# revdotcom/reverb

Measured on NVIDIA H100. Metric: rtfx_attention_rescoring_30s_chunks, higher is better.
Workload: dtype bf16

## Files before the change

reverb_b200/csrc/common.cuh:

```cuda
#pragma once
#include <cuda.h>
#include <cuda_bf16.h>
#include <cuda_runtime.h>
#include <stdint.h>
#include <stdio.h>
#include <string.h>

#include <atomic>

namespace rvb {

void set_error(const char* fmt, ...);
const char* last_error();

#define RVB_CHECK_CUDA(expr)                                                              \
  do {                                                                                    \
    cudaError_t _e = (expr);                                                              \
    if (_e != cudaSuccess) {                                                              \
      rvb::set_error("%s:%d CUDA error %d (%s) in %s", __FILE__, __LINE__, (int)_e,       \
                     cudaGetErrorString(_e), #expr);                                      \
      return -1;                                                                          \
    }                                                                                     \
  } while (0)

#define RVB_REQUIRE(cond, ...)                                                            \
  do {                                                                                    \
    if (!(cond)) {                                                                        \
      rvb::set_error(__VA_ARGS__);                                                        \
      return -2;                                                                          \
    }                                                                                     \
  } while (0)

#define RVB_CHECK_LAUNCH() RVB_CHECK_CUDA(cudaGetLastError())

extern std::atomic<unsigned long long> g_launch_count;
#define RVB_COUNT_LAUNCH() (rvb::g_launch_count.fetch_add(1, std::memory_order_relaxed))

typedef __nv_bfloat16 bf16;

struct DynSmemOptIn {
  static constexpr int kMaxDev = 64;
  std::atomic<size_t> cfg[kMaxDev];
  DynSmemOptIn() {
    for (auto& c : cfg) c.store(0);
  }
  template <typename K>
  int ensure(K kernel, size_t bytes) {
    if (bytes <= 48 * 1024) return 0;
    int dev = 0;
    RVB_CHECK_CUDA(cudaGetDevice(&dev));
    if (dev >= 0 && dev < kMaxDev && cfg[dev].load(std::memory_order_relaxed) >= bytes) return 0;
    RVB_CHECK_CUDA(cudaFuncSetAttribute(kernel, cudaFuncAttributeMaxDynamicSharedMemorySize, (int)bytes));
    if (dev >= 0 && dev < kMaxDev) cfg[dev].store(bytes, std::memory_order_relaxed);
    return 0;
  }
};

__device__ __forceinline__ float2 ffma2(float2 a, float2 b, float2 c) {
  return make_float2(fmaf(a.x, b.x, c.x), fmaf(a.y, b.y, c.y));
}

__device__ __forceinline__ float warp_sum(float v) {
#pragma unroll
  for (int o = 16; o > 0; o >>= 1) v += __shfl_xor_sync(0xffffffffu, v, o);
  return v;
}
__device__ __forceinline__ float warp_max(float v) {
#pragma unroll
  for (int o = 16; o > 0; o >>= 1) v = fmaxf(v, __shfl_xor_sync(0xffffffffu, v, o));
  return v;
}
__device__ __forceinline__ float silu_f(float x) { return x / (1.0f + __expf(-x)); }
__device__ __forceinline__ float sigmoid_f(float x) { return 1.0f / (1.0f + __expf(-x)); }
__device__ __forceinline__ float gelu_erf(float x) { return 0.5f * x * (1.0f + erff(x * 0.70710678118654752f)); }

static inline uint16_t f2bf(float f) {
  uint32_t u;
  memcpy(&u, &f, 4);
  if ((u & 0x7fffffffu) > 0x7f800000u) return (uint16_t)((u >> 16) | 0x40);
  u += 0x7fffu + ((u >> 16) & 1u);
  return (uint16_t)(u >> 16);
}

static inline float bf2f(uint16_t h) {
  uint32_t u = (uint32_t)h << 16;
  float f;
  memcpy(&f, &u, 4);
  return f;
}

__device__ __forceinline__ uint32_t pack_bf16x2(float lo, float hi) {
  __nv_bfloat162 t = __floats2bfloat162_rn(lo, hi);
  return *reinterpret_cast<uint32_t*>(&t);
}
__device__ __forceinline__ float2 unpack_bf16x2(uint32_t u) {
  __nv_bfloat162 t = *reinterpret_cast<__nv_bfloat162*>(&u);
  return __bfloat1622float2(t);
}

__device__ __forceinline__ uint32_t smem_u32(const void* p) {
  return static_cast<uint32_t>(__cvta_generic_to_shared(p));
}

__device__ __forceinline__ void mbar_init(uint64_t* bar, uint32_t count) {
  asm volatile("mbarrier.init.shared::cta.b64 [%0], %1;" ::"r"(smem_u32(bar)), "r"(count));
}
__device__ __forceinline__ void fence_barrier_init() {
  asm volatile("fence.mbarrier_init.release.cluster;" ::: "memory");
}
__device__ __forceinline__ void fence_proxy_async() {
  asm volatile("fence.proxy.async.shared::cta;" ::: "memory");
}
__device__ __forceinline__ void mbar_expect_tx(uint64_t* bar, uint32_t bytes) {
  asm volatile("mbarrier.arrive.expect_tx.shared::cta.b64 _, [%0], %1;" ::"r"(smem_u32(bar)), "r"(bytes)
               : "memory");
}
__device__ __forceinline__ void mbar_arrive(uint64_t* bar) {
  asm volatile("mbarrier.arrive.shared::cta.b64 _, [%0];" ::"r"(smem_u32(bar)) : "memory");
}
__device__ __forceinline__ uint32_t mbar_try_wait(uint64_t* bar, uint32_t parity) {
  uint32_t ok;
  asm volatile(
      "{\n"
      ".reg .pred p;\n"
      "mbarrier.try_wait.parity.shared::cta.b64 p, [%1], %2;\n"
      "selp.u32 %0, 1, 0, p;\n"
      "}\n"
      : "=r"(ok)
      : "r"(smem_u32(bar)), "r"(parity)
      : "memory");
  return ok;
}
__device__ __forceinline__ void mbar_wait(uint64_t* bar, uint32_t parity) {
  while (!mbar_try_wait(bar, parity)) {
  }
}

template <uint32_t N>
__device__ __forceinline__ void setmaxnreg_dec() {
  asm volatile("setmaxnreg.dec.sync.aligned.u32 %0;" ::"n"(N));
}
template <uint32_t N>
__device__ __forceinline__ void setmaxnreg_inc() {
  asm volatile("setmaxnreg.inc.sync.aligned.u32 %0;" ::"n"(N));
}

__device__ __forceinline__ void tma_prefetch_desc(const CUtensorMap* m) {
  asm volatile("prefetch.tensormap [%0];" ::"l"(reinterpret_cast<uint64_t>(m)) : "memory");
}
__device__ __forceinline__ void tma_load_4d(void* smem_dst, const CUtensorMap* m, uint64_t* bar, int c0, int c1,
                                            int c2, int c3) {
  asm volatile(
      "cp.async.bulk.tensor.4d.shared::cluster.global.mbarrier::complete_tx::bytes [%0], [%1, {%3, %4, %5, %6}], [%2];"
      ::"r"(smem_u32(smem_dst)),
      "l"(reinterpret_cast<uint64_t>(m)), "r"(smem_u32(bar)), "r"(c0), "r"(c1), "r"(c2), "r"(c3)
      : "memory");
}
__device__ __forceinline__ void tma_load_2d(void* smem_dst, const CUtensorMap* m, uint64_t* bar, int c0, int c1) {
  asm volatile(
      "cp.async.bulk.tensor.2d.shared::cluster.global.mbarrier::complete_tx::bytes [%0], [%1, {%3, %4}], [%2];"
      ::"r"(smem_u32(smem_dst)),
      "l"(reinterpret_cast<uint64_t>(m)), "r"(smem_u32(bar)), "r"(c0), "r"(c1)
      : "memory");
}

__device__ __forceinline__ void wgmma_fence() { asm volatile("wgmma.fence.sync.aligned;" ::: "memory"); }
__device__ __forceinline__ void wgmma_commit() { asm volatile("wgmma.commit_group.sync.aligned;" ::: "memory"); }
template <int N>
__device__ __forceinline__ void wgmma_wait() {
  asm volatile("wgmma.wait_group.sync.aligned %0;" ::"n"(N) : "memory");
}
template <int R>
__device__ __forceinline__ void wgmma_fence_regs(float* d) {
#pragma unroll
  for (int i = 0; i < R; ++i) asm volatile("" : "+f"(d[i])::"memory");
}
__device__ __forceinline__ void wgmma_m64n128k16_ss(float* d, uint64_t adesc, uint64_t bdesc, uint32_t accumulate) {
  asm volatile(
      "{\n"
      ".reg .pred p;\n"
      "setp.ne.b32 p, %66, 0;\n"
      "wgmma.mma_async.sync.aligned.m64n128k16.f32.bf16.bf16 "
      "{%0, %1, %2, %3, %4, %5, %6, %7, %8, %9, %10, %11, %12, %13, %14, %15, %16, %17, %18, %19, %20, %21, %22, %23, %24, %25, %26, %27, %28, %29, %30, %31, %32, %33, %34, %35, %36, %37, %38, %39, %40, %41, %42, %43, %44, %45, %46, %47, %48, %49, %50, %51, %52, %53, %54, %55, %56, %57, %58, %59, %60, %61, %62, %63}, %64, %65, p, 1, 1, 0, 0;\n"
      "}\n"
      : "+f"(d[0]), "+f"(d[1]), "+f"(d[2]), "+f"(d[3]), "+f"(d[4]), "+f"(d[5]), "+f"(d[6]), "+f"(d[7]), "+f"(d[8]), "+f"(d[9]), "+f"(d[10]), "+f"(d[11]), "+f"(d[12]), "+f"(d[13]), "+f"(d[14]), "+f"(d[15]), "+f"(d[16]), "+f"(d[17]), "+f"(d[18]), "+f"(d[19]), "+f"(d[20]), "+f"(d[21]), "+f"(d[22]), "+f"(d[23]), "+f"(d[24]), "+f"(d[25]), "+f"(d[26]), "+f"(d[27]), "+f"(d[28]), "+f"(d[29]), "+f"(d[30]), "+f"(d[31]), "+f"(d[32]), "+f"(d[33]), "+f"(d[34]), "+f"(d[35]), "+f"(d[36]), "+f"(d[37]), "+f"(d[38]), "+f"(d[39]), "+f"(d[40]), "+f"(d[41]), "+f"(d[42]), "+f"(d[43]), "+f"(d[44]), "+f"(d[45]), "+f"(d[46]), "+f"(d[47]), "+f"(d[48]), "+f"(d[49]), "+f"(d[50]), "+f"(d[51]), "+f"(d[52]), "+f"(d[53]), "+f"(d[54]), "+f"(d[55]), "+f"(d[56]), "+f"(d[57]), "+f"(d[58]), "+f"(d[59]), "+f"(d[60]), "+f"(d[61]), "+f"(d[62]), "+f"(d[63])
      : "l"(adesc), "l"(bdesc), "r"(accumulate)
      : "memory");
}
__device__ __forceinline__ void wgmma_m64n64k16_ss(float* d, uint64_t adesc, uint64_t bdesc, uint32_t accumulate) {
  asm volatile(
      "{\n"
      ".reg .pred p;\n"
      "setp.ne.b32 p, %34, 0;\n"
      "wgmma.mma_async.sync.aligned.m64n64k16.f32.bf16.bf16 "
      "{%0, %1, %2, %3, %4, %5, %6, %7, %8, %9, %10, %11, %12, %13, %14, %15, %16, %17, %18, %19, %20, %21, %22, %23, %24, %25, %26, %27, %28, %29, %30, %31}, %32, %33, p, 1, 1, 0, 0;\n"
      "}\n"
      : "+f"(d[0]), "+f"(d[1]), "+f"(d[2]), "+f"(d[3]), "+f"(d[4]), "+f"(d[5]), "+f"(d[6]), "+f"(d[7]), "+f"(d[8]), "+f"(d[9]), "+f"(d[10]), "+f"(d[11]), "+f"(d[12]), "+f"(d[13]), "+f"(d[14]), "+f"(d[15]), "+f"(d[16]), "+f"(d[17]), "+f"(d[18]), "+f"(d[19]), "+f"(d[20]), "+f"(d[21]), "+f"(d[22]), "+f"(d[23]), "+f"(d[24]), "+f"(d[25]), "+f"(d[26]), "+f"(d[27]), "+f"(d[28]), "+f"(d[29]), "+f"(d[30]), "+f"(d[31])
      : "l"(adesc), "l"(bdesc), "r"(accumulate)
      : "memory");
}
__device__ __forceinline__ void wgmma_m64n64k16_rs_tb(float* d, const uint32_t* a, uint64_t bdesc) {
  asm volatile(
      "wgmma.mma_async.sync.aligned.m64n64k16.f32.bf16.bf16 "
      "{%0, %1, %2, %3, %4, %5, %6, %7, %8, %9, %10, %11, %12, %13, %14, %15, %16, %17, %18, %19, %20, %21, %22, %23, %24, %25, %26, %27, %28, %29, %30, %31}, {%32, %33, %34, %35}, %36, 1, 1, 1, 1;\n"
      : "+f"(d[0]), "+f"(d[1]), "+f"(d[2]), "+f"(d[3]), "+f"(d[4]), "+f"(d[5]), "+f"(d[6]), "+f"(d[7]), "+f"(d[8]), "+f"(d[9]), "+f"(d[10]), "+f"(d[11]), "+f"(d[12]), "+f"(d[13]), "+f"(d[14]), "+f"(d[15]), "+f"(d[16]), "+f"(d[17]), "+f"(d[18]), "+f"(d[19]), "+f"(d[20]), "+f"(d[21]), "+f"(d[22]), "+f"(d[23]), "+f"(d[24]), "+f"(d[25]), "+f"(d[26]), "+f"(d[27]), "+f"(d[28]), "+f"(d[29]), "+f"(d[30]), "+f"(d[31])
      : "r"(a[0]), "r"(a[1]), "r"(a[2]), "r"(a[3]), "l"(bdesc)
      : "memory");
}

__device__ __forceinline__ uint64_t make_sw128_desc(uint32_t smem_addr) {
  uint64_t d = 0;
  d |= (uint64_t)((smem_addr >> 4) & 0x3FFF);
  d |= (uint64_t)(1024 >> 4) << 16;
  d |= (uint64_t)(1024 >> 4) << 32;
  d |= (uint64_t)1 << 62;
  return d;
}

__device__ __forceinline__ uint32_t cluster_ctarank() {
  uint32_t r;
  asm volatile("mov.u32 %0, %%cluster_ctarank;" : "=r"(r));
  return r;
}
__device__ __forceinline__ void cluster_sync_all() {
  asm volatile("barrier.cluster.arrive.release.aligned;\n\tbarrier.cluster.wait.acquire.aligned;" ::: "memory");
}

}
```

reverb_b200/csrc/gemm.cu:

```cuda
#include <cuda.h>
#include <stdlib.h>
#include <string.h>

#include <algorithm>
#include <mutex>
#include <vector>

#include "kernels.h"

namespace rvb {

static int g_gemm_impl = -1;
void set_gemm_impl(int impl) { g_gemm_impl = impl; }
int get_gemm_impl() {
  if (g_gemm_impl < 0) {
    const char* e = getenv("RVB_GEMM");
    g_gemm_impl = (e && strcmp(e, "simt") == 0) ? 1 : (e && strcmp(e, "narrow") == 0) ? 2 : 0;
  }
  return g_gemm_impl;
}

struct GemmKParams {
  int M, N, K, num_k_blocks;
  int tiles_n, num_tiles;
// ... 480 lines not shown
          }
          if (EPI == EPI_BF16_RELU) {
#pragma unroll
            for (int e = 0; e < 8; ++e) v[e] = fmaxf(v[e], 0.f);
          }
          if (EPI == EPI_BF16_GELU) {
#pragma unroll
            for (int e = 0; e < 8; ++e) v[e] = gelu_erf(v[e]);
          }
          if constexpr (EPI == EPI_BF16_RELPOS) {
            if (kcols) {
              const uint4 pv = *reinterpret_cast<const uint4*>(p.rp_pos + (long long)rp_t * p.rp_ldp + rp_hc + 8 * j);
              const float4 u0 = __ldg(reinterpret_cast<const float4*>(p.rp_u + rp_hc + 8 * j));
              const float4 u1 = __ldg(reinterpret_cast<const float4*>(p.rp_u + rp_hc + 8 * j) + 1);
              const float uu[8] = {u0.x, u0.y, u0.z, u0.w, u1.x, u1.y, u1.z, u1.w};
              const float4 v0 = __ldg(reinterpret_cast<const float4*>(p.rp_v + rp_hc + 8 * j));
              const float4 v1 = __ldg(reinterpret_cast<const float4*>(p.rp_v + rp_hc + 8 * j) + 1);
              const float2 p0 = unpack_bf16x2(pv.x), p1 = unpack_bf16x2(pv.y), p2 = unpack_bf16x2(pv.z), p3 = unpack_bf16x2(pv.w);
              const float pp[8] = {p0.x, p0.y, p1.x, p1.y, p2.x, p2.y, p3.x, p3.y};
              float kq[8];
#pragma unroll
              for (int e = 0; e < 8; ++e) {
                kq[e] = __bfloat162float(__float2bfloat16(v[e]));
                v[e] = kq[e] + pp[e];
              }
              rp_part[j] = uu[0] * kq[0] + uu[1] * kq[1] + uu[2] * kq[2] + uu[3] * kq[3] + uu[4] * kq[4] + uu[5] * kq[5] +
                           uu[6] * kq[6] + uu[7] * kq[7] + v0.x * pp[0] + v0.y * pp[1] + v0.z * pp[2] + v0.w * pp[3] +
                           v1.x * pp[4] + v1.y * pp[5] + v1.z * pp[6] + v1.w * pp[7];
            }
          }
          if (PAIR && part == 1) {
#pragma unroll
            for (int e = 0; e < 8; ++e) v[e] -= __bfloat162float(__float2bfloat16(v[e]));
          }
          if (p.debug_skip_epi == 3 && v[0] != 123.456f) continue;
          *reinterpret_cast<uint4*>(stage_u + lane * 32 + ((j ^ (lane & 7)) << 2)) =
              make_uint4(pack_bf16x2(v[0], v[1]), pack_bf16x2(v[2], v[3]), pack_bf16x2(v[4], v[5]),
                         pack_bf16x2(v[6], v[7]));
        }
        if (p.debug_skip_epi == 3) continue;
        __syncwarp();
#pragma unroll
        for (int it = 0; it < 8; ++it) {
          const int row = it * 4 + rsub;
          const uint4 u = *reinterpret_cast<const uint4*>(stage_u + row * 32 + ((slot ^ (row & 7)) << 2));
          if (ro[it] >= 0 && p.debug_skip_epi != 2)
            *reinterpret_cast<uint4*>(out + ro[it] + c + (PAIR ? part * p.out_split : 0)) = u;
        }
        __syncwarp();
        }
        if constexpr (EPI == EPI_BF16_RELPOS) {
          if (kcols && orow >= 0) {
            const int hh = rp_hc >> 6;
            p.rp_cb[((orow / p.rp_T) * p.rp_H + hh) * (long long)p.rp_T + rp_t] =
                ((rp_part[0] + rp_part[4]) + (rp_part[2] + rp_part[6])) + ((rp_part[1] + rp_part[5]) + (rp_part[3] + rp_part[7]));
          }
        }
      } else {
        for (int cc = c; cc < c + 64 && cc < c1; cc += 32) {
          if (n0_tile + cc >= p.N) break;
          uint32_t acc[32];
          acc_ld32<BN>(accs, arow, cc, acc);
          if (orow >= 0) store_chunk<EPI>(p, orow, n0_tile + cc, oshift, acc);
        }
      }
    }
  } else if ((EPI == EPI_RESID || EPI == EPI_F32) && p.f32_coalesced) {
    const int slot = lane & 7, rsub = lane >> 3;
    long long ro[8];
#pragma unroll
    for (int it = 0; it < 8; ++it) {
      const long long o = __shfl_sync(0xffffffffu, orow, it * 4 + rsub);
      ro[it] = (o >= 0) ? o * p.ldo + n0_tile - oshift + slot * 4 : -1;
    }
    float* out = reinterpret_cast<float*>(p.out);
    float4 r[8];
    if (EPI == EPI_RESID && n0_tile + c0 + slot * 4 + 4 <= p.N) {
#pragma unroll
      for (int it = 0; it < 8; ++it)
        if (ro[it] >= 0) r[it] = *reinterpret_cast<const float4*>(out + ro[it] + c0);
    }
#pragma unroll 1
    for (int c = c0; c < c1; c += 32) {
      if (n0_tile + c >= p.N) break;
      uint32_t acc[32];
      acc_ld32<BN>(accs, arow, c, acc);
      const int n = n0_tile + c + slot * 4;
      const bool vec = (n + 4 <= p.N);
      float4 rn[8];
      const bool pre_next = EPI == EPI_RESID && (c + 32 < c1) && (n + 32 + 4 <= p.N);
      if (pre_next) {
#pragma unroll
        for (int it = 0; it < 8; ++it)
          if (ro[it] >= 0) rn[it] = *reinterpret_cast<const float4*>(out + ro[it] + c + 32);
      }
      float4 b4 = make_float4(0.f, 0.f, 0.f, 0.f);
      if (p.bias != nullptr) {
        if (vec) {
          b4 = __ldg(reinterpret_cast<const float4*>(p.bias + n));
        } else {
          if (n + 0 < p.N) b4.x = __ldg(p.bias + n + 0);
          if (n + 1 < p.N) b4.y = __ldg(p.bias + n + 1);
          if (n + 2 < p.N) b4.z = __ldg(p.bias + n + 2);
        }
      }
#pragma unroll
      for (int j = 0; j < 8; ++j)
        *reinterpret_cast<uint4*>(stage + lane * 32 + ((j ^ (lane & 7)) << 2)) =
            make_uint4(acc[4 * j], acc[4 * j + 1], acc[4 * j + 2], acc[4 * j + 3]);
      __syncwarp();
#pragma unroll
      for (int it = 0; it < 8; ++it) {
        const int row = it * 4 + rsub;
        float4 v = *reinterpret_cast<const float4*>(stage + row * 32 + ((slot ^ (row & 7)) << 2));
        v.x += b4.x; v.y += b4.y; v.z += b4.z; v.w += b4.w;
        if (ro[it] < 0) continue;
        float* o = out + ro[it] + c;
        if (vec) {
          if (EPI == EPI_RESID) {
            r[it].x += p.alpha * v.x; r[it].y += p.alpha * v.y; r[it].z += p.alpha * v.z; r[it].w += p.alpha * v.w;
            *reinterpret_cast<float4*>(o) = r[it];
          } else {
            *reinterpret_cast<float4*>(o) = v;
          }
        } else {
          const float vv[4] = {v.x, v.y, v.z, v.w};
#pragma unroll
          for (int k = 0; k < 3; ++k)
            if (n + k < p.N) o[k] = (EPI == EPI_RESID) ? o[k] + p.alpha * vv[k] : vv[k];
        }
      }
      __syncwarp();
      if (pre_next) {
#pragma unroll
        for (int it = 0; it < 8; ++it) r[it] = rn[it];
      }
    }
  } else {
#pragma unroll 1
    for (int c = c0; c < c1; c += 32) {
      if (n0_tile + c >= p.N) break;
      uint32_t acc[32];
      acc_ld32<BN>(accs, arow, c, acc);
      if (orow >= 0) store_chunk<EPI>(p, orow, n0_tile + c, oshift, acc);
    }
  }
}

constexpr int kConsumerWGs = 2;
constexpr int kGemmThreads = 128 * (1 + kConsumerWGs);
constexpr int kProducerRegs = 40;
constexpr int kConsumerRegs = 232;

template <int BN>
struct GemmCfg {
  static constexpr int BM = 128;
  static constexpr int BK = 64;
  static constexpr int STAGES = 4;
  static constexpr uint32_t A_BYTES = BM * BK * 2;
  static constexpr uint32_t B_BYTES = BN * BK * 2;
  static constexpr uint32_t STAGE_BYTES = A_BYTES + B_BYTES;
  static constexpr uint32_t ACC_BYTES = BM * BN * 4;
  static constexpr uint32_t SMEM_BYTES = STAGES * STAGE_BYTES + ACC_BYTES + 4 * 4096  +
                                         256  + 1024 ;
};

template <int BN, int EPI, bool PAIR>
__global__ void __launch_bounds__(kGemmThreads, 1)
gemm_wg_kernel(const __grid_constant__ CUtensorMap tmA, const __grid_constant__ CUtensorMap tmB, const GemmKParams p) {
  using Cfg = GemmCfg<BN>;
  constexpr int STAGES = Cfg::STAGES;
  extern __shared__ uint8_t smem_raw[];
  uint8_t* smem = reinterpret_cast<uint8_t*>((reinterpret_cast<uintptr_t>(smem_raw) + 1023) & ~uintptr_t(1023));
  uint8_t* sA = smem;
  uint8_t* sB = smem + STAGES * Cfg::A_BYTES;
  float* accs = reinterpret_cast<float*>(smem + STAGES * Cfg::STAGE_BYTES);
  float* stage_epi = accs + Cfg::BM * BN;
  uint64_t* bars = reinterpret_cast<uint64_t*>(stage_epi + 4 * 1024);
  uint64_t* full = bars;
  uint64_t* empty = bars + STAGES;
  uint64_t* turn = bars + 2 * STAGES;
  uint64_t* accfree = turn + 2;

  const int warp = threadIdx.x >> 5;
  const int lane = threadIdx.x & 31;

  if (threadIdx.x == 0) {
    for (int i = 0; i < STAGES; ++i) {
      mbar_init(&full[i], 1);
      mbar_init(&empty[i], 4);
    }
    for (int w = 0; w < kConsumerWGs; ++w) {
      mbar_init(&turn[w], 128);
      mbar_init(&accfree[w], 128);
    }
    fence_barrier_init();
    tma_prefetch_desc(&tmA);
    tma_prefetch_desc(&tmB);
  }
  __syncthreads();
  const int nkb = p.num_k_blocks;

  if (warp < 4) {
    setmaxnreg_dec<kProducerRegs>();
    if (warp == 0 && lane == 0) {
      uint32_t stage = 0, phase = 0;
      for (int tile = blockIdx.x; tile < p.num_tiles; tile += gridDim.x) {
        if (!tile_active(p, tile, BN)) continue;
        TileCoord t = decode_tile(p, tile, BN);
        for (int kbx = 0; kbx < nkb; ++kbx) {
          const int seg = p.x3 ? kbx / p.kb_seg : 0;
          const int kb = kbx - seg * p.kb_seg;
          const int a_ofs = (seg == 1) ? p.a_lo_ofs : 0, w_ofs = (seg == 2) ? p.w_lo_ofs : 0;
          mbar_wait(&empty[stage], phase ^ 1);
          mbar_expect_tx(&full[stage], Cfg::STAGE_BYTES);
          if (p.conv_mode) {
            int tap = kb / p.conv_cblocks;
            int cb = kb - tap * p.conv_cblocks;
            int kh = tap / 3, kw = tap - kh * 3;
            tma_load_4d(sA + stage * Cfg::A_BYTES, &tmA, &full[stage], cb * 64 + a_ofs, 2 * t.f + kw, t.row0 + (kh >> 1),
                        t.b * 2 + (kh & 1));
          } else {
            tma_load_4d(sA + stage * Cfg::A_BYTES, &tmA, &full[stage], kb * 64 + a_ofs, t.row0, 0, 0);
          }
          tma_load_2d(sB + stage * Cfg::B_BYTES, &tmB, &full[stage], kb * 64 + w_ofs, t.n0);
          if (++stage == STAGES) {
            stage = 0;
            phase ^= 1;
          }
        }
      }
    }
  } else {
    setmaxnreg_inc<kConsumerRegs>();
    const int wg = (warp >> 2) - 1, wl = warp & 3;
    float* stage_w = stage_epi + wl * 1024;
    float acc[BN];
    int active = 0;
    for (int tile = blockIdx.x; tile < p.num_tiles; tile += gridDim.x) {
      if (!tile_active(p, tile, BN)) continue;
      const int i = active++;
      if (i % kConsumerWGs != wg) continue;
      TileCoord t = decode_tile(p, tile, BN);
      const uint32_t u0 = (uint32_t)i * (uint32_t)nkb;
      uint32_t stage = u0 % STAGES, phase = (u0 / STAGES) & 1;
      const uint32_t hand_parity = ((i - 1) >> 1) & 1;
#pragma unroll
      for (int e = 0; e < BN; ++e) acc[e] = 0.f;
      if (i > 0) mbar_wait(&turn[wg], hand_parity);
      int prev = -1;
      for (int kb = 0; kb < nkb; ++kb) {
        mbar_wait(&full[stage], phase);
        const uint64_t adesc = make_sw128_desc(smem_u32(sA + stage * Cfg::A_BYTES));
        const uint64_t bdesc = make_sw128_desc(smem_u32(sB + stage * Cfg::B_BYTES));
        constexpr uint64_t kHalfA = (Cfg::A_BYTES / 2) >> 4;
        wgmma_fence_regs<BN>(acc);
        wgmma_fence();
#pragma unroll
        for (int k = 0; k < 4; ++k) {
          if constexpr (BN == 128) {
            wgmma_m64n128k16_ss(acc, adesc + 2 * k, bdesc + 2 * k, 1u);
            wgmma_m64n128k16_ss(acc + BN / 2, adesc + kHalfA + 2 * k, bdesc + 2 * k, 1u);
          } else {
            wgmma_m64n64k16_ss(acc, adesc + 2 * k, bdesc + 2 * k, 1u);
            wgmma_m64n64k16_ss(acc + BN / 2, adesc + kHalfA + 2 * k, bdesc + 2 * k, 1u);
          }
        }
        wgmma_commit();
        wgmma_wait<1>();
        wgmma_fence_regs<BN>(acc);
        if (prev >= 0 && lane == 0) mbar_arrive(&empty[prev]);
        prev = (int)stage;
        if (++stage == STAGES) {
          stage = 0;
          phase ^= 1;
        }
      }
      mbar_arrive(&turn[wg ^ 1]);
      wgmma_wait<0>();
      wgmma_fence_regs<BN>(acc);
      if (prev >= 0 && lane == 0) mbar_arrive(&empty[prev]);
      if (i > 0) mbar_wait(&accfree[wg], hand_parity);
#pragma unroll
      for (int h = 0; h < 2; ++h) {
        const int r0 = h * 64 + wl * 16 + (lane >> 2);
#pragma unroll
        for (int j = 0; j < BN / 8; ++j) {
          const int c = 8 * j + 2 * (lane & 3);
#pragma unroll
          for (int e = 0; e < 2; ++e) {
            const int r = r0 + 8 * e;
            *reinterpret_cast<float2*>(accs + r * BN + ((((c >> 2)) ^ (r & 7)) << 2) + (c & 3)) =
                make_float2(acc[h * (BN / 2) + 4 * j + 2 * e], acc[h * (BN / 2) + 4 * j + 2 * e + 1]);
          }
        }
      }
      asm volatile("bar.sync %0, 128;" ::"r"(1 + wg) : "memory");
      drain_tile<BN, EPI, PAIR>(p, t, wl, lane, accs, 0, BN, stage_w);
      mbar_arrive(&accfree[wg ^ 1]);
    }
  }
}

__device__ __forceinline__ float load_a_elem(const GemmKParams& p, const TileCoord& t, int r, int k) {
  if (k >= p.K) return 0.0f;
  if (p.conv_mode) {
    int tp = t.row0 + r;
    if (tp >= p.conv_T2) return 0.0f;
    int tap = k / p.conv_C;
    int c = k - tap * p.conv_C;
    int kh = tap / 3, kw = tap - kh * 3;
    long long idx = (((long long)(t.b * 2 + (kh & 1)) * p.conv_T1h + (tp + (kh >> 1))) * p.conv_F1 + (2 * t.f + kw)) *
                        p.conv_C + c;
    return __bfloat162float(p.A[idx]);
  }
  int m = t.row0 + r;
  if (m >= p.M) return 0.0f;
  return __bfloat162float(p.A[(long long)m * p.lda + k]);
}

__global__ void __launch_bounds__(256) gemm_simt_kernel(const GemmKParams p) {
  __shared__ float sA[128][17];
  __shared__ float sW[32][17];
  __shared__ float sG[32][17];
  const bool glu = (p.act == ACT_GLU);
  for (int tile = blockIdx.x; tile < p.num_tiles; tile += gridDim.x) {
    TileCoord t = decode_tile(p, tile, 32);
    const int tx = threadIdx.x & 7, ty = threadIdx.x >> 3;
    const int wrow0 = glu ? 2 * t.n0 : t.n0;
    float acc[4][4], accg[4][4];
#pragma unroll
    for (int i = 0; i < 4; ++i)
#pragma unroll
      for (int j = 0; j < 4; ++j) acc[i][j] = accg[i][j] = 0.f;
    for (int k0 = 0; k0 < p.K; k0 += 16) {
      for (int e = threadIdx.x; e < 128 * 16; e += 256) {
        int r = e >> 4, kk = e & 15;
        sA[r][kk] = load_a_elem(p, t, r, k0 + kk);
      }
      for (int e = threadIdx.x; e < 32 * 16; e += 256) {
        int n = e >> 4, kk = e & 15;
        int gn = wrow0 + n, gk = k0 + kk;
        sW[n][kk] = (gn < p.N && gk < p.K) ? __bfloat162float(p.W[(long long)gn * p.ldw + gk]) : 0.f;
        sG[n][kk] = (glu && gn + 32 < p.N && gk < p.K) ? __bfloat162float(p.W[(long long)(gn + 32) * p.ldw + gk]) : 0.f;
      }
      __syncthreads();
#pragma unroll
      for (int kk = 0; kk < 16; ++kk) {
        float a[4], w[4], g[4];
#pragma unroll
        for (int i = 0; i < 4; ++i) a[i] = sA[ty * 4 + i][kk];
#pragma unroll
        for (int j = 0; j < 4; ++j) {
          w[j] = sW[tx * 4 + j][kk];
          g[j] = sG[tx * 4 + j][kk];
        }
#pragma unroll
        for (int i = 0; i < 4; ++i)
#pragma unroll
          for (int j = 0; j < 4; ++j) {
            acc[i][j] = fmaf(a[i], w[j], acc[i][j]);
            accg[i][j] = fmaf(a[i], g[j], accg[i][j]);
          }
      }
      __syncthreads();
    }
    for (int i = 0; i < 4; ++i) {
      long long orow = output_row(p, t, ty * 4 + i);
      if (orow < 0) continue;
      for (int j = 0; j < 4; ++j) {
        int n = t.n0 + tx * 4 + j;
        if (glu) {
          if (2 * n >= p.N) continue;
          const int wr = wrow0 + tx * 4 + j;
          float va = acc[i][j], vg = accg[i][j];
          if (p.bias) {
            va += p.bias[wr];
            vg += p.bias[wr + 32];
          }
          reinterpret_cast<bf16*>(p.out)[orow * p.ldo + n] = __float2bfloat16(va / (1.f + expf(-vg)));
          continue;
        }
        if (n >= p.N) continue;
        float x = acc[i][j];
        if (p.bias) x += p.bias[n];
        x = apply_act(x, p.act);
        if (p.out_mode == OUT_BF16)
          reinterpret_cast<bf16*>(p.out)[orow * p.ldo + n] = __float2bfloat16(x);
        else if (p.out_mode == OUT_F32)
          reinterpret_cast<float*>(p.out)[orow * p.ldo + n] = x;
        else
          reinterpret_cast<float*>(p.out)[orow * p.ldo + n] += p.alpha * x;
      }
    }
  }
}

typedef CUresult (*EncodeTiledFn)(CUtensorMap*, CUtensorMapDataType, cuuint32_t, void*, const cuuint64_t*,
                                  const cuuint64_t*, const cuuint32_t*, const cuuint32_t*, CUtensorMapInterleave,
                                  CUtensorMapSwizzle, CUtensorMapL2promotion, CUtensorMapFloatOOBfill);
static EncodeTiledFn g_encode = nullptr;

static int get_encode_fn() {
  if (g_encode) return 0;
  void* fn = nullptr;
  cudaDriverEntryPointQueryResult qres;
  RVB_CHECK_CUDA(cudaGetDriverEntryPoint("cuTensorMapEncodeTiled", &fn, cudaEnableDefault, &qres));
  RVB_REQUIRE(fn != nullptr && qres == cudaDriverEntryPointSuccess, "cuTensorMapEncodeTiled not available");
  g_encode = reinterpret_cast<EncodeTiledFn>(fn);
  return 0;
}

static int make_tmap(CUtensorMap* m, const void* base, int rank, const cuuint64_t* dims, const cuuint64_t* strides_bytes,
                     const cuuint32_t* box) {
  cuuint32_t estr[5] = {1, 1, 1, 1, 1};
  CUresult r = g_encode(m, CU_TENSOR_MAP_DATA_TYPE_BFLOAT16, rank, const_cast<void*>(base), dims, strides_bytes, box,
                        estr, CU_TENSOR_MAP_INTERLEAVE_NONE, CU_TENSOR_MAP_SWIZZLE_128B,
                        CU_TENSOR_MAP_L2_PROMOTION_L2_256B, CU_TENSOR_MAP_FLOAT_OOB_FILL_NONE);
  RVB_REQUIRE(r == CUDA_SUCCESS, "cuTensorMapEncodeTiled failed with %d (rank %d dims %llu %llu)", (int)r, rank,
              (unsigned long long)dims[0], (unsigned long long)dims[1]);
  return 0;
}

static int g_num_sms = 0;

struct GemmProfRec {
  cudaEvent_t a, b;
  double flops;
};
static bool g_prof_on = false;
static std::vector<GemmProfRec> g_prof;
static std::mutex g_prof_mutex;
constexpr int kProfMaxDev = 64;
static std::vector<cudaEvent_t> g_prof_pool[kProfMaxDev];
static size_t g_prof_pool_used[kProfMaxDev];

static int prof_event(cudaEvent_t* out) {
  int dev = 0;
  RVB_CHECK_CUDA(cudaGetDevice(&dev));
  RVB_REQUIRE(dev >= 0 && dev < kProfMaxDev, "gemm profile: device index %d out of range", dev);
  std::lock_guard<std::mutex> lock(g_prof_mutex);
  auto& pool = g_prof_pool[dev];
  if (g_prof_pool_used[dev] == pool.size()) {
    cudaEvent_t e;
    RVB_CHECK_CUDA(cudaEventCreate(&e));
    pool.push_back(e);
  }
  *out = pool[g_prof_pool_used[dev]++];
  return 0;
}

void gemm_profile_begin() {
  std::lock_guard<std::mutex> lock(g_prof_mutex);
  g_prof.clear();
  for (int d = 0; d < kProfMaxDev; ++d) g_prof_pool_used[d] = 0;
  g_prof_on = true;
}
int gemm_profile_end(double* total_ms, double* total_flops, long long* launches) {
  g_prof_on = false;
  double ms = 0.0, fl = 0.0;
  for (auto& r : g_prof) {
    float t = 0.f;
    RVB_CHECK_CUDA(cudaEventSynchronize(r.b));
    RVB_CHECK_CUDA(cudaEventElapsedTime(&t, r.a, r.b));
    ms += t;
    fl += r.flops;
  }
  if (total_ms) *total_ms = ms;
  if (total_flops) *total_flops = fl;
  if (launches) *launches = (long long)g_prof.size();
  g_prof.clear();
  return 0;
}

template <int BN>
static int launch_wg(const GemmArgs& a, GemmKParams& p, cudaStream_t stream) {
  using Cfg = GemmCfg<BN>;
  CUtensorMap tmA, tmB;
  const int kmul = a.x3 ? 2 : 1;
  const long long lda = a.lda ? a.lda : (long long)a.K * kmul, ldw = a.ldw ? a.ldw : (long long)a.K * kmul;
  if (a.conv_mode) {
    const cuuint64_t Cp = (cuuint64_t)a.conv_C * (a.x3 ? 2 : 1);
    cuuint64_t dims[4] = {Cp, (cuuint64_t)a.conv_F1, (cuuint64_t)a.conv_T1h, (cuuint64_t)(2 * a.conv_B)};
    cuuint64_t str[3] = {Cp * 2, (cuuint64_t)a.conv_F1 * Cp * 2, (cuuint64_t)a.conv_T1h * a.conv_F1 * Cp * 2};
    cuuint32_t box[4] = {64, 1, 128, 1};
    if (make_tmap(&tmA, a.A, 4, dims, str, box)) return -1;
  } else {
    cuuint64_t dims[4] = {(cuuint64_t)a.K * (a.x3 ? 2 : 1), (cuuint64_t)a.M, 1, 1};
    cuuint64_t str[3] = {(cuuint64_t)lda * 2, (cuuint64_t)lda * 2 * a.M, (cuuint64_t)lda * 2 * a.M};
    cuuint32_t box[4] = {64, 128, 1, 1};
    if (make_tmap(&tmA, a.A, 4, dims, str, box)) return -1;
  }
  {
    cuuint64_t dims[2] = {(cuuint64_t)a.K * (a.x3 ? 2 : 1), (cuuint64_t)a.N};
    cuuint64_t str[1] = {(cuuint64_t)ldw * 2};
    cuuint32_t box[2] = {64, (cuuint32_t)BN};
    if (make_tmap(&tmB, a.W, 2, dims, str, box)) return -1;
  }
  void (*kern)(const CUtensorMap, const CUtensorMap, const GemmKParams) = nullptr;
  const bool pair = a.out_split > 0;
  switch (a.rp_pos ? (int)EPI_BF16_RELPOS : select_epi(a.act, a.out_mode)) {
    case EPI_BF16: kern = pair ? gemm_wg_kernel<BN, EPI_BF16, true> : gemm_wg_kernel<BN, EPI_BF16, false>; break;
    case EPI_BF16_RELU: kern = pair ? gemm_wg_kernel<BN, EPI_BF16_RELU, true> : gemm_wg_kernel<BN, EPI_BF16_RELU, false>; break;
    case EPI_BF16_SILU: kern = pair ? gemm_wg_kernel<BN, EPI_BF16_SILU, true> : gemm_wg_kernel<BN, EPI_BF16_SILU, false>; break;
    case EPI_F32: kern = gemm_wg_kernel<BN, EPI_F32, false>; break;
    case EPI_RESID: kern = gemm_wg_kernel<BN, EPI_RESID, false>; break;
    case EPI_GLU: kern = pair ? gemm_wg_kernel<BN, EPI_GLU, true> : gemm_wg_kernel<BN, EPI_GLU, false>; break;
    case EPI_LSE: kern = gemm_wg_kernel<BN, EPI_LSE, false>; break;
    case EPI_BF16_RELPOS: kern = gemm_wg_kernel<BN, EPI_BF16_RELPOS, false>; break;
    case EPI_BF16_GELU: kern = gemm_wg_kernel<BN, EPI_BF16_GELU, false>; break;
    default: kern = gemm_wg_kernel<BN, EPI_GENERIC, false>; break;
  }
  RVB_CHECK_CUDA(cudaFuncSetAttribute(kern, cudaFuncAttributeMaxDynamicSharedMemorySize, (int)Cfg::SMEM_BYTES));
  p.tiles_n = a.grp ? p.grp_slots * (p.group_n / BN) : (a.N + BN - 1) / BN;
  int tiles_m = a.conv_mode ? a.conv_B * a.conv_F2 * p.conv_tt : (a.M + 127) / 128;
  p.num_tiles = tiles_m * p.tiles_n;
  int grid = p.num_tiles < g_num_sms ? p.num_tiles : g_num_sms;
  GemmProfRec rec;
  if (g_prof_on) {
    if (prof_event(&rec.a) || prof_event(&rec.b)) return -1;
    rec.flops = 2.0 * (double)a.M * (double)(a.grp ? a.group_n : a.N) * (double)a.K * (a.x3 ? 3.0 : 1.0);
    RVB_CHECK_CUDA(cudaEventRecord(rec.a, stream));
  }
  kern<<<grid, kGemmThreads, Cfg::SMEM_BYTES, stream>>>(tmA, tmB, p);
  RVB_COUNT_LAUNCH();
  RVB_CHECK_LAUNCH();
  if (g_prof_on) {
    RVB_CHECK_CUDA(cudaEventRecord(rec.b, stream));
    {
      std::lock_guard<std::mutex> lock(g_prof_mutex);
      g_prof.push_back(rec);
    }
  }
  return 0;
}

int launch_gemm(const GemmArgs& a, cudaStream_t stream) {
  RVB_REQUIRE(a.A && a.W && (a.out || a.out_mode == OUT_LSE), "gemm: null pointer");
  RVB_REQUIRE(a.M > 0 && a.N > 0 && a.K > 0, "gemm: bad shape M=%d N=%d K=%d", a.M, a.N, a.K);
  if (g_num_sms == 0) {
    int dev = 0;
    RVB_CHECK_CUDA(cudaGetDevice(&dev));
    RVB_CHECK_CUDA(cudaDeviceGetAttribute(&g_num_sms, cudaDevAttrMultiProcessorCount, dev));
  }
  GemmKParams p;
  memset(&p, 0, sizeof(p));
  p.M = a.M;
  p.N = a.N;
  p.K = a.K;
  p.num_k_blocks = (a.K + 63) / 64;
  p.x3 = a.x3;
  p.kb_seg = p.num_k_blocks;
  p.out_split = a.out_split;
  if (a.x3) {
    RVB_REQUIRE(a.K % 64 == 0, "gemm: bf16x3 mode needs K %% 64 == 0 (K=%d)", a.K);
    RVB_REQUIRE(get_gemm_impl() != 1, "gemm: bf16x3 mode is not built for the simt bring-up kernel");
    p.num_k_blocks *= 3;
    p.a_lo_ofs = a.conv_mode ? a.conv_C : a.K;
    p.w_lo_ofs = a.K;
  }
  if (a.out_split > 0)
    RVB_REQUIRE((a.out_mode == OUT_BF16) && a.out_split % 8 == 0, "gemm: out_split needs an aligned bf16 output");
  p.bias = a.bias;
  p.act = a.act;
  p.out_mode = a.out_mode;
  p.out = a.out;
  if (a.grp) {
    RVB_REQUIRE(a.group_n > 0 && a.group_n % 64 == 0 && a.N % a.group_n == 0 && a.rows_per_batch > 0 &&
                    a.act == ACT_NONE && (a.out_mode == OUT_BF16 || a.out_mode == OUT_F32) && !a.conv_mode && !a.rp_pos,
                "gemm: a grouped output needs group_n %% 64 == 0 dividing N (N=%d group_n=%d), rows_per_batch, no "
                "activation and a plain bf16 / fp32 output", a.N, a.group_n);
    RVB_REQUIRE(get_gemm_impl() != 1, "gemm: grouped output is not built for the simt bring-up kernel");
  }
  p.grp = a.grp;
  p.group_n = a.grp ? a.group_n : a.N;
  if (a.grp) {
    const int rpb = a.rows_per_batch, n_utt = (a.M + rpb - 1) / rpb;
    p.grp_slots = std::min(n_utt, 127 / rpb + 2);
  }
  p.ldo = a.ldo ? a.ldo : (long long)(a.act == ACT_GLU ? a.N / 2 : p.group_n) * (a.out_split > 0 ? 2 : 1);
  p.alpha = a.alpha;
  p.row_lens = a.row_lens;
  p.rows_per_batch = a.rows_per_batch > 0 ? a.rows_per_batch : a.M;
  p.conv_mode = a.conv_mode;
  p.lse_gather = a.lse_gather;
  p.lse_part = a.lse_part;
  p.lse_tgt = a.lse_tgt;
  p.lse_nslab = lse_slabs(a.N);
  p.rp_pos = a.rp_pos;
  p.rp_ldp = a.rp_ldp;
  p.rp_T = a.rp_T;
  p.rp_H = a.rp_H;
  p.rp_col0 = a.rp_col0;
  p.rp_u = a.rp_u;
  p.rp_v = a.rp_v;
  p.rp_cb = a.rp_cb;
  if (a.rp_pos) {
    RVB_REQUIRE(a.out_mode == OUT_BF16 && a.act == ACT_NONE && a.out_split == 0 && !a.conv_mode && a.rp_T > 0 &&
                    a.rp_col0 % 64 == 0 && a.rp_ldp % 8 == 0 && a.N % 64 == 0 && a.rp_u && a.rp_v && a.rp_cb &&
                    (reinterpret_cast<uintptr_t>(a.rp_pos) & 15) == 0 && (reinterpret_cast<uintptr_t>(a.rp_u) & 15) == 0 &&
                    (reinterpret_cast<uintptr_t>(a.rp_v) & 15) == 0,
                "gemm: rel-pos epilogue needs a plain bf16 output, 64-aligned key columns and 16-byte aligned tables");
    RVB_REQUIRE(get_gemm_impl() != 1, "gemm: rel-pos epilogue is not built for the simt bring-up kernel");
  }
  if (a.act == ACT_GELU) {
    RVB_REQUIRE(a.out_mode == OUT_BF16 && a.out_split == 0 && !a.x3 && !a.grp && !a.rp_pos,
                "gemm: ACT_GELU needs a plain bf16 output");
    RVB_REQUIRE(get_gemm_impl() != 1, "gemm: ACT_GELU is not built for the simt bring-up kernel");
  }
  if (a.out_mode == OUT_LSE) {
    RVB_REQUIRE(a.lse_gather && a.lse_part && a.lse_tgt && a.act == ACT_NONE && !a.conv_mode && a.N > 128,
                "gemm: OUT_LSE needs gather / partial / target buffers, no activation and N > 128");
    RVB_REQUIRE(get_gemm_impl() != 1, "gemm: OUT_LSE is not built for the simt bring-up kernel");
  }
  {
    static int skip = -1;
    if (skip < 0) {
      const char* e = getenv("RVB_GEMM_SKIP_EPI");
      skip = e ? atoi(e) : 0;
    }
    p.debug_skip_epi = skip;
  }
  p.glu_coalesced = (a.act == ACT_GLU);
  p.bf16_coalesced = (a.out_mode == OUT_BF16) && (a.act != ACT_GLU) && (p.ldo % 8 == 0) &&
                     ((reinterpret_cast<uintptr_t>(a.out) & 15) == 0) &&
                     (a.bias == nullptr || (reinterpret_cast<uintptr_t>(a.bias) & 15) == 0);
  p.f32_coalesced = (a.out_mode != OUT_BF16) && (p.ldo % 4 == 0) && ((reinterpret_cast<uintptr_t>(a.out) & 15) == 0) &&
                    (a.bias == nullptr || (reinterpret_cast<uintptr_t>(a.bias) & 15) == 0);
  p.A = a.A;
  p.W = a.W;
  p.lda = a.lda ? a.lda : (long long)a.K * (a.x3 ? 2 : 1);
  p.ldw = a.ldw ? a.ldw : (long long)a.K * (a.x3 ? 2 : 1);
  if (a.conv_mode) {
    RVB_REQUIRE(a.conv_C % 64 == 0, "conv implicit GEMM needs C %% 64 == 0 (C=%d)", a.conv_C);
    RVB_REQUIRE(a.K == 9 * a.conv_C && a.M == a.conv_B * a.conv_F2 * a.conv_T2, "conv implicit GEMM: bad M/K");
    p.conv_T2 = a.conv_T2;
    p.conv_F2 = a.conv_F2;
    p.conv_orow_mul = a.conv_pair_out ? 2 * a.conv_F2 : a.conv_F2;
    p.conv_tt = (a.conv_T2 + 127) / 128;
    p.conv_cblocks = a.conv_C / 64;
    p.conv_T1h = a.conv_T1h;
    p.conv_F1 = a.conv_F1;
    p.conv_C = a.conv_C;
  }
  if (a.out_split > 0)
    RVB_REQUIRE(a.N % 128 == 0 && (a.act == ACT_GLU ? p.glu_coalesced : p.bf16_coalesced),
                "gemm: a hi/lo output pair needs N %% 128 == 0 and 16-byte aligned rows (N=%d)", a.N);
  if (a.act == ACT_GLU) {
    RVB_REQUIRE(a.out_mode == OUT_BF16 && a.N % 64 == 0 && !a.conv_mode, "gemm: ACT_GLU needs bf16 output and N %% 64 == 0");
    RVB_REQUIRE((reinterpret_cast<uintptr_t>(a.out) & 15) == 0 && p.ldo % 8 == 0 &&
                    (a.bias == nullptr || (reinterpret_cast<uintptr_t>(a.bias) & 15) == 0),
                "gemm: ACT_GLU needs 16-byte aligned output rows and bias");
  }
  if (get_gemm_impl() == 1) {
    p.tiles_n = ((a.act == ACT_GLU ? a.N / 2 : a.N) + 31) / 32;
    int tiles_m = a.conv_mode ? a.conv_B * a.conv_F2 * p.conv_tt : (a.M + 127) / 128;
    p.num_tiles = tiles_m * p.tiles_n;
    int grid = p.num_tiles < g_num_sms * 8 ? p.num_tiles : g_num_sms * 8;
    gemm_simt_kernel<<<grid, 256, 0, stream>>>(p);
    RVB_COUNT_LAUNCH();
    RVB_CHECK_LAUNCH();
    return 0;
  }
  RVB_REQUIRE((reinterpret_cast<uintptr_t>(a.A) & 15) == 0 && (reinterpret_cast<uintptr_t>(a.W) & 15) == 0,
              "gemm: operands must be 16-byte aligned");
  RVB_REQUIRE((p.lda * 2) % 16 == 0 && (p.ldw * 2) % 16 == 0, "gemm: leading dimensions must be multiples of 8");
  if (get_encode_fn()) return -1;
  const bool narrow = p.group_n <= 64 || (get_gemm_impl() == 2 && a.out_mode != OUT_LSE && !(a.act == ACT_GLU && a.out_split > 0));
  RVB_REQUIRE(!a.grp || p.group_n % (narrow ? 64 : 128) == 0, "gemm: grouped output needs group_n %% %d == 0 (group_n=%d)",
              narrow ? 64 : 128, p.group_n);
  if (!narrow) return launch_wg<128>(a, p, stream);
  return launch_wg<64>(a, p, stream);
}

}
```

Measured before the change: 12310.

## Add 128x256 wide-tile warp-specialized GEMM kernel for simple bf16 epilogues

Adds a new GEMM kernel using m64n256k16 wgmma with 128x256 output tiles, a 3-stage TMA pipeline, and a dedicated store path where three producer-side warps write the smem-staged output to global memory. The dispatcher routes non-grouped, non-paired bf16/ReLU/SiLU GEMMs to it when N is a multiple of 256 and there are at least as many tiles as SMs. The wider tile raises operand reuse per loaded A block and lowers B/A traffic ratio, while overlapping epilogue stores with the next tile's MMA. The cost is 128 accumulator registers per thread, fewer pipeline stages, and a possible load-balance loss on mid-sized shapes.

```diff
diff --git a/reverb_b200/csrc/common.cuh b/reverb_b200/csrc/common.cuh
--- a/reverb_b200/csrc/common.cuh
+++ b/reverb_b200/csrc/common.cuh
@@ -175,6 +175,18 @@
 #pragma unroll
   for (int i = 0; i < R; ++i) asm volatile("" : "+f"(d[i])::"memory");
 }
+__device__ __forceinline__ void wgmma_m64n256k16_ss(float* d, uint64_t adesc, uint64_t bdesc, uint32_t accumulate) {
+  asm volatile(
+      "{\n"
+      ".reg .pred p;\n"
+      "setp.ne.b32 p, %130, 0;\n"
+      "wgmma.mma_async.sync.aligned.m64n256k16.f32.bf16.bf16 "
+      "{%0, %1, %2, %3, %4, %5, %6, %7, %8, %9, %10, %11, %12, %13, %14, %15, %16, %17, %18, %19, %20, %21, %22, %23, %24, %25, %26, %27, %28, %29, %30, %31, %32, %33, %34, %35, %36, %37, %38, %39, %40, %41, %42, %43, %44, %45, %46, %47, %48, %49, %50, %51, %52, %53, %54, %55, %56, %57, %58, %59, %60, %61, %62, %63, %64, %65, %66, %67, %68, %69, %70, %71, %72, %73, %74, %75, %76, %77, %78, %79, %80, %81, %82, %83, %84, %85, %86, %87, %88, %89, %90, %91, %92, %93, %94, %95, %96, %97, %98, %99, %100, %101, %102, %103, %104, %105, %106, %107, %108, %109, %110, %111, %112, %113, %114, %115, %116, %117, %118, %119, %120, %121, %122, %123, %124, %125, %126, %127}, %128, %129, p, 1, 1, 0, 0;\n"
+      "}\n"
+      : "+f"(d[0]), "+f"(d[1]), "+f"(d[2]), "+f"(d[3]), "+f"(d[4]), "+f"(d[5]), "+f"(d[6]), "+f"(d[7]), "+f"(d[8]), "+f"(d[9]), "+f"(d[10]), "+f"(d[11]), "+f"(d[12]), "+f"(d[13]), "+f"(d[14]), "+f"(d[15]), "+f"(d[16]), "+f"(d[17]), "+f"(d[18]), "+f"(d[19]), "+f"(d[20]), "+f"(d[21]), "+f"(d[22]), "+f"(d[23]), "+f"(d[24]), "+f"(d[25]), "+f"(d[26]), "+f"(d[27]), "+f"(d[28]), "+f"(d[29]), "+f"(d[30]), "+f"(d[31]), "+f"(d[32]), "+f"(d[33]), "+f"(d[34]), "+f"(d[35]), "+f"(d[36]), "+f"(d[37]), "+f"(d[38]), "+f"(d[39]), "+f"(d[40]), "+f"(d[41]), "+f"(d[42]), "+f"(d[43]), "+f"(d[44]), "+f"(d[45]), "+f"(d[46]), "+f"(d[47]), "+f"(d[48]), "+f"(d[49]), "+f"(d[50]), "+f"(d[51]), "+f"(d[52]), "+f"(d[53]), "+f"(d[54]), "+f"(d[55]), "+f"(d[56]), "+f"(d[57]), "+f"(d[58]), "+f"(d[59]), "+f"(d[60]), "+f"(d[61]), "+f"(d[62]), "+f"(d[63]), "+f"(d[64]), "+f"(d[65]), "+f"(d[66]), "+f"(d[67]), "+f"(d[68]), "+f"(d[69]), "+f"(d[70]), "+f"(d[71]), "+f"(d[72]), "+f"(d[73]), "+f"(d[74]), "+f"(d[75]), "+f"(d[76]), "+f"(d[77]), "+f"(d[78]), "+f"(d[79]), "+f"(d[80]), "+f"(d[81]), "+f"(d[82]), "+f"(d[83]), "+f"(d[84]), "+f"(d[85]), "+f"(d[86]), "+f"(d[87]), "+f"(d[88]), "+f"(d[89]), "+f"(d[90]), "+f"(d[91]), "+f"(d[92]), "+f"(d[93]), "+f"(d[94]), "+f"(d[95]), "+f"(d[96]), "+f"(d[97]), "+f"(d[98]), "+f"(d[99]), "+f"(d[100]), "+f"(d[101]), "+f"(d[102]), "+f"(d[103]), "+f"(d[104]), "+f"(d[105]), "+f"(d[106]), "+f"(d[107]), "+f"(d[108]), "+f"(d[109]), "+f"(d[110]), "+f"(d[111]), "+f"(d[112]), "+f"(d[113]), "+f"(d[114]), "+f"(d[115]), "+f"(d[116]), "+f"(d[117]), "+f"(d[118]), "+f"(d[119]), "+f"(d[120]), "+f"(d[121]), "+f"(d[122]), "+f"(d[123]), "+f"(d[124]), "+f"(d[125]), "+f"(d[126]), "+f"(d[127])
+      : "l"(adesc), "l"(bdesc), "r"(accumulate)
+      : "memory");
+}
 __device__ __forceinline__ void wgmma_m64n128k16_ss(float* d, uint64_t adesc, uint64_t bdesc, uint32_t accumulate) {
   asm volatile(
       "{\n"
diff --git a/reverb_b200/csrc/gemm.cu b/reverb_b200/csrc/gemm.cu
--- a/reverb_b200/csrc/gemm.cu
+++ b/reverb_b200/csrc/gemm.cu
@@ -806,6 +806,153 @@
   }
 }
 
+struct WideCfg {
+  static constexpr int BM = 128;
+  static constexpr int BN = 256;
+  static constexpr int BK = 64;
+  static constexpr int STAGES = 3;
+  static constexpr uint32_t A_BYTES = BM * BK * 2;
+  static constexpr uint32_t B_BYTES = BN * BK * 2;
+  static constexpr uint32_t STAGE_BYTES = A_BYTES + B_BYTES;
+  static constexpr uint32_t OUT_BYTES = BM * BN * 2;
+  static constexpr uint32_t SMEM_BYTES = STAGES * STAGE_BYTES + OUT_BYTES + 256  + 1024 ;
+};
+
+template <int EPI>
+__global__ void __launch_bounds__(kGemmThreads, 1)
+gemm_wide_kernel(const __grid_constant__ CUtensorMap tmA, const __grid_constant__ CUtensorMap tmB, const GemmKParams p) {
+  using Cfg = WideCfg;
+  constexpr int STAGES = Cfg::STAGES;
+  extern __shared__ uint8_t smem_raw[];
+  uint8_t* smem = reinterpret_cast<uint8_t*>((reinterpret_cast<uintptr_t>(smem_raw) + 1023) & ~uintptr_t(1023));
+  uint8_t* sA = smem;
+  uint8_t* sB = smem + STAGES * Cfg::A_BYTES;
+  uint8_t* sOut = smem + STAGES * Cfg::STAGE_BYTES;
+  uint64_t* bars = reinterpret_cast<uint64_t*>(sOut + Cfg::OUT_BYTES);
+  uint64_t* full = bars;
+  uint64_t* empty = bars + STAGES;
+  uint64_t* ofull = bars + 2 * STAGES;
+  uint64_t* ofree = ofull + 1;
+
+  const int warp = threadIdx.x >> 5;
+  const int lane = threadIdx.x & 31;
+
+  if (threadIdx.x == 0) {
+    for (int i = 0; i < STAGES; ++i) {
+      mbar_init(&full[i], 1);
+      mbar_init(&empty[i], 8);
+    }
+    mbar_init(ofull, 256);
+    mbar_init(ofree, 96);
+    fence_barrier_init();
+    tma_prefetch_desc(&tmA);
+    tma_prefetch_desc(&tmB);
+  }
+  __syncthreads();
+  const int nkb = p.num_k_blocks;
+
+  if (warp < 4) {
+    setmaxnreg_dec<kProducerRegs>();
+    if (warp == 0) {
+      if (lane == 0) {
+        uint32_t stage = 0, phase = 0;
+        for (int tile = blockIdx.x; tile < p.num_tiles; tile += gridDim.x) {
+          const TileCoord t = decode_tile(p, tile, Cfg::BN);
+          for (int kb = 0; kb < nkb; ++kb) {
+            mbar_wait(&empty[stage], phase ^ 1);
+            mbar_expect_tx(&full[stage], Cfg::STAGE_BYTES);
+            if (p.conv_mode) {
+              const int tap = kb / p.conv_cblocks;
+              const int cb = kb - tap * p.conv_cblocks;
+              const int kh = tap / 3, kw = tap - kh * 3;
+              tma_load_4d(sA + stage * Cfg::A_BYTES, &tmA, &full[stage], cb * 64, 2 * t.f + kw, t.row0 + (kh >> 1),
+                          t.b * 2 + (kh & 1));
+            } else {
+              tma_load_4d(sA + stage * Cfg::A_BYTES, &tmA, &full[stage], kb * 64, t.row0, 0, 0);
+            }
+            tma_load_2d(sB + stage * Cfg::B_BYTES, &tmB, &full[stage], kb * 64, t.n0);
+            if (++stage == STAGES) {
+              stage = 0;
+              phase ^= 1;
+            }
+          }
+        }
+      }
+    } else {
+      const int cw = warp - 1;
+      const bool store = p.debug_skip_epi == 0;
+      bf16* out = reinterpret_cast<bf16*>(p.out);
+      int i = 0;
+      for (int tile = blockIdx.x; tile < p.num_tiles; tile += gridDim.x, ++i) {
+        const TileCoord t = decode_tile(p, tile, Cfg::BN);
+        mbar_wait(ofull, i & 1);
+        if (store) {
+#pragma unroll 4
+          for (int r = cw; r < Cfg::BM; r += 3) {
+            const long long orow = output_row(p, t, r);
+            const uint4 u = *reinterpret_cast<const uint4*>(sOut + r * (Cfg::BN * 2) + ((lane ^ (r & 7)) << 4));
+            if (orow >= 0) *reinterpret_cast<uint4*>(out + orow * p.ldo + t.n0 + lane * 8) = u;
+          }
+        }
+        mbar_arrive(ofree);
+      }
+    }
+  } else {
+    setmaxnreg_inc<kConsumerRegs>();
+    const int wg = (warp >> 2) - 1, wl = warp & 3;
+    float acc[Cfg::BN / 2];
+    uint32_t stage = 0, phase = 0;
+    int i = 0;
+    for (int tile = blockIdx.x; tile < p.num_tiles; tile += gridDim.x, ++i) {
+      const TileCoord t = decode_tile(p, tile, Cfg::BN);
+#pragma unroll
+      for (int e = 0; e < Cfg::BN / 2; ++e) acc[e] = 0.f;
+      int prev = -1;
+      for (int kb = 0; kb < nkb; ++kb) {
+        mbar_wait(&full[stage], phase);
+        constexpr uint64_t kHalfA = (Cfg::A_BYTES / 2) >> 4;
+        const uint64_t adesc = make_sw128_desc(smem_u32(sA + stage * Cfg::A_BYTES)) + wg * kHalfA;
+        const uint64_t bdesc = make_sw128_desc(smem_u32(sB + stage * Cfg::B_BYTES));
+        wgmma_fence_regs<Cfg::BN / 2>(acc);
+        wgmma_fence();
+#pragma unroll
+        for (int k = 0; k < 4; ++k) wgmma_m64n256k16_ss(acc, adesc + 2 * k, bdesc + 2 * k, 1u);
+        wgmma_commit();
+        wgmma_wait<1>();
+        wgmma_fence_regs<Cfg::BN / 2>(acc);
+        if (prev >= 0 && lane == 0) mbar_arrive(&empty[prev]);
+        prev = (int)stage;
+        if (++stage == STAGES) {
+          stage = 0;
+          phase ^= 1;
+        }
+      }
+      wgmma_wait<0>();
+      wgmma_fence_regs<Cfg::BN / 2>(acc);
+      if (lane == 0) mbar_arrive(&empty[prev]);
+      if (i > 0) mbar_wait(ofree, (i - 1) & 1);
+      if (p.debug_skip_epi != 1) {
+        const int r0 = wg * 64 + wl * 16 + (lane >> 2);
+        uint32_t* so = reinterpret_cast<uint32_t*>(sOut) + r0 * (Cfg::BN / 2) + (lane & 3);
+        const float2 one2 = make_float2(1.f, 1.f);
+#pragma unroll
+        for (int j = 0; j < Cfg::BN / 8; ++j) {
+          float2 b = make_float2(0.f, 0.f);
+          if (p.bias != nullptr) b = __ldg(reinterpret_cast<const float2*>(p.bias + t.n0 + 8 * j + 2 * (lane & 3)));
+#pragma unroll
+          for (int e = 0; e < 2; ++e) {
+            float2 v = ffma2(make_float2(acc[4 * j + 2 * e], acc[4 * j + 2 * e + 1]), one2, b);
+            if (EPI == EPI_BF16_SILU) v = gated2(v, v);
+            if (EPI == EPI_BF16_RELU) v = make_float2(fmaxf(v.x, 0.f), fmaxf(v.y, 0.f));
+            so[8 * e * (Cfg::BN / 2) + ((j ^ (lane >> 2)) << 2)] = pack_bf16x2(v.x, v.y);
+          }
+        }
+      }
+      mbar_arrive(ofull);
+    }
+  }
+}
+
 __device__ __forceinline__ float load_a_elem(const GemmKParams& p, const TileCoord& t, int r, int k) {
   if (k >= p.K) return 0.0f;
   if (p.conv_mode) {
@@ -979,7 +1126,7 @@
 
 template <int BN>
 static int launch_wg(const GemmArgs& a, GemmKParams& p, cudaStream_t stream) {
-  using Cfg = GemmCfg<BN>;
+  constexpr uint32_t SMEM_BYTES = BN == 256 ? WideCfg::SMEM_BYTES : GemmCfg<BN>::SMEM_BYTES;
   CUtensorMap tmA, tmB;
   const int kmul = a.x3 ? 2 : 1;
   const long long lda = a.lda ? a.lda : (long long)a.K * kmul, ldw = a.ldw ? a.ldw : (long long)a.K * kmul;
@@ -1002,20 +1149,28 @@
     if (make_tmap(&tmB, a.W, 2, dims, str, box)) return -1;
   }
   void (*kern)(const CUtensorMap, const CUtensorMap, const GemmKParams) = nullptr;
-  const bool pair = a.out_split > 0;
-  switch (a.rp_pos ? (int)EPI_BF16_RELPOS : select_epi(a.act, a.out_mode)) {
-    case EPI_BF16: kern = pair ? gemm_wg_kernel<BN, EPI_BF16, true> : gemm_wg_kernel<BN, EPI_BF16, false>; break;
-    case EPI_BF16_RELU: kern = pair ? gemm_wg_kernel<BN, EPI_BF16_RELU, true> : gemm_wg_kernel<BN, EPI_BF16_RELU, false>; break;
-    case EPI_BF16_SILU: kern = pair ? gemm_wg_kernel<BN, EPI_BF16_SILU, true> : gemm_wg_kernel<BN, EPI_BF16_SILU, false>; break;
-    case EPI_F32: kern = gemm_wg_kernel<BN, EPI_F32, false>; break;
-    case EPI_RESID: kern = gemm_wg_kernel<BN, EPI_RESID, false>; break;
-    case EPI_GLU: kern = pair ? gemm_wg_kernel<BN, EPI_GLU, true> : gemm_wg_kernel<BN, EPI_GLU, false>; break;
-    case EPI_LSE: kern = gemm_wg_kernel<BN, EPI_LSE, false>; break;
-    case EPI_BF16_RELPOS: kern = gemm_wg_kernel<BN, EPI_BF16_RELPOS, false>; break;
-    case EPI_BF16_GELU: kern = gemm_wg_kernel<BN, EPI_BF16_GELU, false>; break;
-    default: kern = gemm_wg_kernel<BN, EPI_GENERIC, false>; break;
-  }
-  RVB_CHECK_CUDA(cudaFuncSetAttribute(kern, cudaFuncAttributeMaxDynamicSharedMemorySize, (int)Cfg::SMEM_BYTES));
+  if constexpr (BN == 256) {
+    switch (select_epi(a.act, a.out_mode)) {
+      case EPI_BF16: kern = gemm_wide_kernel<EPI_BF16>; break;
+      case EPI_BF16_RELU: kern = gemm_wide_kernel<EPI_BF16_RELU>; break;
+      default: kern = gemm_wide_kernel<EPI_BF16_SILU>; break;
+    }
+  } else {
+    const bool pair = a.out_split > 0;
+    switch (a.rp_pos ? (int)EPI_BF16_RELPOS : select_epi(a.act, a.out_mode)) {
+      case EPI_BF16: kern = pair ? gemm_wg_kernel<BN, EPI_BF16, true> : gemm_wg_kernel<BN, EPI_BF16, false>; break;
+      case EPI_BF16_RELU: kern = pair ? gemm_wg_kernel<BN, EPI_BF16_RELU, true> : gemm_wg_kernel<BN, EPI_BF16_RELU, false>; break;
+      case EPI_BF16_SILU: kern = pair ? gemm_wg_kernel<BN, EPI_BF16_SILU, true> : gemm_wg_kernel<BN, EPI_BF16_SILU, false>; break;
+      case EPI_F32: kern = gemm_wg_kernel<BN, EPI_F32, false>; break;
+      case EPI_RESID: kern = gemm_wg_kernel<BN, EPI_RESID, false>; break;
+      case EPI_GLU: kern = pair ? gemm_wg_kernel<BN, EPI_GLU, true> : gemm_wg_kernel<BN, EPI_GLU, false>; break;
+      case EPI_LSE: kern = gemm_wg_kernel<BN, EPI_LSE, false>; break;
+      case EPI_BF16_RELPOS: kern = gemm_wg_kernel<BN, EPI_BF16_RELPOS, false>; break;
+      case EPI_BF16_GELU: kern = gemm_wg_kernel<BN, EPI_BF16_GELU, false>; break;
+      default: kern = gemm_wg_kernel<BN, EPI_GENERIC, false>; break;
+    }
+  }
+  RVB_CHECK_CUDA(cudaFuncSetAttribute(kern, cudaFuncAttributeMaxDynamicSharedMemorySize, (int)SMEM_BYTES));
   p.tiles_n = a.grp ? p.grp_slots * (p.group_n / BN) : (a.N + BN - 1) / BN;
   int tiles_m = a.conv_mode ? a.conv_B * a.conv_F2 * p.conv_tt : (a.M + 127) / 128;
   p.num_tiles = tiles_m * p.tiles_n;
@@ -1026,7 +1181,7 @@
     rec.flops = 2.0 * (double)a.M * (double)(a.grp ? a.group_n : a.N) * (double)a.K * (a.x3 ? 3.0 : 1.0);
     RVB_CHECK_CUDA(cudaEventRecord(rec.a, stream));
   }
-  kern<<<grid, kGemmThreads, Cfg::SMEM_BYTES, stream>>>(tmA, tmB, p);
+  kern<<<grid, kGemmThreads, SMEM_BYTES, stream>>>(tmA, tmB, p);
   RVB_COUNT_LAUNCH();
   RVB_CHECK_LAUNCH();
   if (g_prof_on) {
@@ -1173,8 +1328,15 @@
   const bool narrow = p.group_n <= 64 || (get_gemm_impl() == 2 && a.out_mode != OUT_LSE && !(a.act == ACT_GLU && a.out_split > 0));
   RVB_REQUIRE(!a.grp || p.group_n % (narrow ? 64 : 128) == 0, "gemm: grouped output needs group_n %% %d == 0 (group_n=%d)",
               narrow ? 64 : 128, p.group_n);
-  if (!narrow) return launch_wg<128>(a, p, stream);
-  return launch_wg<64>(a, p, stream);
-}
-
-}
+  if (narrow) return launch_wg<64>(a, p, stream);
+  const int epi = select_epi(a.act, a.out_mode);
+  const long long wide_tiles = (long long)(a.conv_mode ? a.conv_B * a.conv_F2 * p.conv_tt : (a.M + 127) / 128) * (a.N / 256);
+  const char* wide_env = getenv("RVB_GEMM_WIDE");
+  if ((epi == EPI_BF16 || epi == EPI_BF16_RELU || epi == EPI_BF16_SILU) && !a.rp_pos && !a.grp && !a.x3 &&
+      a.out_split == 0 && p.bf16_coalesced && a.N % 256 == 0 && wide_tiles >= g_num_sms &&
+      !(wide_env && strcmp(wide_env, "0") == 0))
+    return launch_wg<256>(a, p, stream);
+  return launch_wg<128>(a, p, stream);
+}
+
+}
```

Result: faster. 12990 (median of 6 runs) (+5.6%).
